# opendilab/DI-engine

Hardware: NVIDIA H100
Metric: learner transitions/sec (GAE+ppo_error fwd+bwd, T=128 x B=4096 per GPU) (higher is better)
Workload: dtype f32

## Files before the change

### di-engine_b200/_lib.py

```python
import ctypes
import os
from ctypes import c_double, c_int, c_longlong, c_size_t, c_void_p

_HERE = os.path.dirname(os.path.abspath(__file__))
LIB_PATH = os.environ.get("B200RL_LIB") or os.path.join(_HERE, "lib", "libb200rl.so")

P = c_void_p
LL = c_longlong
D = c_double
I = c_int

PROTOTYPES = {
    "b200rl_version": [],
    "b200rl_built_for_sm": [],
    "b200rl_workspace_bytes": [],
    "b200rl_gae": [P, P, P, P, P, P, LL, LL, LL, D, D, I, P],
    "b200rl_gae_returns": [P, P, P, P, P, LL, LL, LL, D, D, I, D, P, P, P, P, P, P, P, c_size_t, P],
    "b200rl_adv_stats": [P, LL, P, P, c_size_t, P],
    "b200rl_normalize": [P, P, LL, P, P],
    "b200rl_gae_returns_norm": [P, P, P, P, P, LL, LL, D, D, I, D, P, P, P, P, P, P, P, P, P, c_size_t, P],
    "b200rl_value_map_fwd": [I, P, LL, P, P],
    "b200rl_value_map_bwd": [I, P, P, LL, P, P],
    "b200rl_impala_mask": [P, P, P, LL, LL, P, P, P, P],
    "b200rl_ppo_fwd": [P, P, P, P, P, P, P, P, P, LL, LL, LL, D, I, D, I, P, P, P, P, c_size_t, P],
    "b200rl_ppo_bwd": [P, P, P, P, P, P, P, P, P, LL, LL, LL, D, I, D, I, P, P, P, P, P, P, P, P, P, P, P],
    "b200rl_ppo_fwd_grad": [P, P, P, P, P, P, P, P, P, LL, LL, LL, D, I, D, I, P, P, P, P, P, P, P, P, c_size_t, P],
    "b200rl_ppo_value_fwd": [P, P, P, P, LL, D, I, P, P, P, c_size_t, P],
    "b200rl_ppo_fused_supported": [P, P, P, P, P, P, P, P, P, P, LL, LL],
    "b200rl_ppo_tile_geometry": [LL, LL, I, I, I, I, P],
    "b200rl_qntd_fwd": [P, P, P, P, P, P, P, P, LL, P, LL, LL, LL, I, D, I, I, D, I, D, I, LL, D, P, P, P, P, P, P, P,
                        c_size_t, P],
    "b200rl_qntd_bwd": [P, P, P, P, P, LL, LL, LL, I, LL, I, P, P],
    "b200rl_dqfd_fwd": [P, P, P, P, P, P, P, P, P, P, P, LL, P, LL, LL, I, D, I, I, D, I, D, D, D, D, D, LL, D, P, P, P,
                        P, P, P, P, P, P, c_size_t, P],
    "b200rl_dqfd_bwd": [P, P, P, P, P, P, P, P, LL, LL, D, D, D, LL, I, P, P],
    "b200rl_soft_td_fwd": [I, P, P, P, P, P, P, P, P, LL, LL, LL, LL, I, D, D, D, I, I, D, P, P, P, P, P, P, P, P, P,
                           c_size_t, P],
    "b200rl_dntd_fwd":[P, P, P, P, P, P, P, LL, P, LL, P, LL, LL, LL, I, I, D, D, D, P, P, P, P, P, P, c_size_t, P],
    "b200rl_dntd_bwd": [P, P, P, P, LL, P, P, LL, LL, I, I, P, P],
    "b200rl_lambda_returns": [P, P, P, D, P, D, P, I, LL, LL, P, P],
    "b200rl_lambda_returns_bwd": [P, P, P, P, P, D, P, D, P, I, LL, LL, P, P, P, P, P],
    "b200rl_tb_cross_entropy_fwd": [P, P, P, LL, LL, LL, P, P],
    "b200rl_tb_cross_entropy_bwd": [P, P, P, P, LL, LL, LL, P, P],
    "b200rl_td_lambda_fwd": [P, P, P, D, D, LL, LL, P, P, P, c_size_t, P],
    "b200rl_scale": [P, P, P, LL, P],
    "b200rl_upgo_head_fwd": [P, P, P, P, P, P, LL, LL, LL, P, P, P, P, c_size_t, P],
    "b200rl_upgo_head_bwd": [P, P, P, P, P, LL, LL, LL, I, P, P],
    "b200rl_vtrace_fwd": [P, P, P, P, P, P, LL, LL, LL, D, D, D, D, D, P, P, P, P, P, c_size_t, P],
    "b200rl_vtrace_continuous_fwd": [P, P, P, P, P, P, P, P, LL, LL, LL, D, D, D, D, D, P, P, P, P, P, c_size_t, P],
    "b200rl_vtrace_continuous_bwd": [P, P, P, P, P, P, P, P, P, LL, LL, LL, P, P, P, P],
# ... 76 lines not shown
```

### di-engine_b200/csrc/gae_tile.cuh

```cuda
#pragma once
#include "common.cuh"

namespace b200rl {

template <int ID, int COUNT>
__device__ __forceinline__ void named_bar_sync() {
    asm volatile("bar.sync %0, %1;" ::"n"(ID), "n"(COUNT) : "memory");
}
template <int ID, int COUNT>
__device__ __forceinline__ void named_bar_arrive() {
    asm volatile("bar.arrive %0, %1;" ::"n"(ID), "n"(COUNT) : "memory");
}
template <int COUNT>
__device__ __forceinline__ void chunk_arrive(int k) {
    if (k == 0) named_bar_arrive<1, COUNT>();
    else if (k == 1) named_bar_arrive<2, COUNT>();
    else if (k == 2) named_bar_arrive<3, COUNT>();
    else named_bar_arrive<4, COUNT>();
}
__device__ __forceinline__ void scanned_arrive(int k) {
    if (k == 0) named_bar_arrive<5, 64>();
    else if (k == 1) named_bar_arrive<6, 64>();
    else if (k == 2) named_bar_arrive<7, 64>();
    else named_bar_arrive<8, 64>();
}
__device__ __forceinline__ void scanned_wait(int k) {
    if (k == 0) named_bar_sync<5, 64>();
    else if (k == 1) named_bar_sync<6, 64>();
    else if (k == 2) named_bar_sync<7, 64>();
    else named_bar_sync<8, 64>();
}
template <int COUNT>
__device__ __forceinline__ void chunk_wait(int k) {
    if (k == 0) named_bar_sync<1, COUNT>();
    else if (k == 1) named_bar_sync<2, COUNT>();
    else if (k == 2) named_bar_sync<3, COUNT>();
    else named_bar_sync<4, COUNT>();
}

constexpr int GAE_CH = 32;
constexpr int GAE_NCHUNK = 4;
constexpr int GAE_SLAB = GAE_CH * GAE_NCHUNK;

template <int TC, bool VEC, class OnChunk>
__device__ __forceinline__ void gae_tile_body(
    const float* __restrict__ value, float* __restrict__ next_value, const float* __restrict__ reward,
    const float* __restrict__ done, const float* __restrict__ traj, float* __restrict__ adv, long long T,
    long long C, long long A, float gamma, float gl, int mask_inplace, long long c0,
    float (*s_d)[GAE_CH][TC], float (*s_f)[GAE_CH][TC], OnChunk on_chunk_done, float vscale = 0.f) {
    constexpr int NL = (TC / 4) * 32;
    constexpr int NTHREADS = NL + 32;
    const long long Caux = C / A;
    const bool is_scan = threadIdx.x < 32;
    const int ltid = threadIdx.x - 32;
    float carry = 0.f;
    for (long long hi = T; hi > 0; hi -= GAE_SLAB) {
        const long long lo = hi > GAE_SLAB ? hi - GAE_SLAB : 0;
        const int rows = (int)(hi - lo);
        if (!is_scan) {
            if (VEC) {
                constexpr int TPR = TC / 4;
                const int cq = (ltid % TPR) * 4;
                const int rr = ltid / TPR;
                const long long c = c0 + cq;
                const bool col_ok = c < C;
                constexpr int DEPTH = 2;
                float4 v[DEPTH], nv[DEPTH], rw[DEPTH], dn[DEPTH], tf[DEPTH];
                auto issue = [&](int k, int b) {
                    const int r = rows - 1 - k * GAE_CH - rr;
                    if (r >= 0 && col_ok) {
                        const long long off = (lo + r) * C + c;
                        v[b] = ldg_stream4(reinterpret_cast<const float4*>(value + off));
                        nv[b] = ldg_stream4(reinterpret_cast<const float4*>(next_value + off));
                        rw[b] = ldg_stream4(reinterpret_cast<const float4*>(reward + off));
                        dn[b] = done ? ldg_stream4(reinterpret_cast<const float4*>(done + off))
                                     : make_float4(0.f, 0.f, 0.f, 0.f);
                        tf[b] = traj ? ldg_stream4(reinterpret_cast<const float4*>(traj + off)) : dn[b];
                    }
                };
#pragma unroll
                for (int k = 0; k < DEPTH; ++k) issue(k, k);
#pragma unroll
                for (int k = 0; k < GAE_NCHUNK; ++k) {
                    const int b = k % DEPTH;
                    const int r = rows - 1 - k * GAE_CH - rr;
                    if (r >= 0 && col_ok) {
                        float vv[4] = {v[b].x, v[b].y, v[b].z, v[b].w}, nn[4] = {nv[b].x, nv[b].y, nv[b].z, nv[b].w};
                        float rw4[4] = {rw[b].x, rw[b].y, rw[b].z, rw[b].w};
                        float dd[4] = {dn[b].x, dn[b].y, dn[b].z, dn[b].w};
                        float tt[4] = {tf[b].x, tf[b].y, tf[b].z, tf[b].w};
                        float de[4], fa[4];
                        bool changed = false;
#pragma unroll
                        for (int q = 0; q < 4; ++q) {
                            if (vscale != 0.f) {
                                vv[q] = fmul(vv[q], vscale);
                                nn[q] = fmul(nn[q], vscale);
                            }
                            if (done) {
                                changed |= (dd[q] != 0.f);
                                nn[q] = fmul(nn[q], fsub(1.f, dd[q]));
                            }
                            de[q] = fsub(fadd(rw4[q], fmul(gamma, nn[q])), vv[q]);
                            fa[q] = fmul(gl, fsub(1.f, tt[q]));
                        }
                        *reinterpret_cast<float4*>(&s_d[k][rr][cq]) = make_float4(de[0], de[1], de[2], de[3]);
                        *reinterpret_cast<float4*>(&s_f[k][rr][cq]) = make_float4(fa[0], fa[1], fa[2], fa[3]);
                        if (changed && mask_inplace)
                            *reinterpret_cast<float4*>(next_value + (lo + r) * C + c) =
                                make_float4(nn[0], nn[1], nn[2], nn[3]);
                    }
                    chunk_arrive<NTHREADS>(k);
                    if (k + DEPTH < GAE_NCHUNK) issue(k + DEPTH, b);
                }
            } else {
#pragma unroll
                for (int k = 0; k < GAE_NCHUNK; ++k) {
                    const int rtop = rows - 1 - k * GAE_CH;
                    for (int i = ltid; i < GAE_CH * TC; i += NL) {
                        const int rr = i / TC, cc = i % TC;
                        const int r = rtop - rr;
                        const long long c = c0 + cc;
                        if (r >= 0 && c < C) {
                            const long long off = (lo + r) * C + c;
                            const long long aoff = (lo + r) * Caux + c / A;
                            float nvv = next_value[off];
                            if (vscale != 0.f) nvv = fmul(nvv, vscale);
                            const float dnn = done ? done[aoff] : 0.f;
                            const float tff = traj ? traj[aoff] : dnn;
                            if (done) {
                                const float mm = fmul(nvv, fsub(1.f, dnn));
                                if (mask_inplace && dnn != 0.f) next_value[off] = mm;
                                nvv = mm;
                            }
                            const float vvv = vscale != 0.f ? fmul(value[off], vscale) : value[off];
                            s_d[k][rr][cc] = fsub(fadd(reward[aoff], fmul(gamma, nvv)), vvv);
                            s_f[k][rr][cc] = fmul(gl, fsub(1.f, tff));
                        }
                    }
                    chunk_arrive<NTHREADS>(k);
                }
            }
        } else {
            const int cc = threadIdx.x;
            const bool lane_ok = cc < TC && c0 + cc < C;
#pragma unroll 1
            for (int k = 0; k < GAE_NCHUNK; ++k) {
                chunk_wait<NTHREADS>(k);
                const int rtop = rows - 1 - k * GAE_CH;
                if (lane_ok && rtop >= 0) {
                    if (rtop >= GAE_CH - 1) {
                        float d[GAE_CH], f[GAE_CH];
#pragma unroll
                        for (int j = 0; j < GAE_CH; ++j) {
                            d[j] = s_d[k][j][cc];
                            f[j] = s_f[k][j][cc];
                        }
#pragma unroll
                        for (int j = 0; j < GAE_CH; ++j) {
                            carry = fadd(d[j], fmul(f[j], carry));
                            s_d[k][j][cc] = carry;
                        }
                    } else {
                        for (int j = 0; j <= rtop; ++j) {
                            carry = fadd(s_d[k][j][cc], fmul(s_f[k][j][cc], carry));
                            s_d[k][j][cc] = carry;
                        }
                    }
                }
                scanned_arrive(k);
// ... 36 lines not shown
```

### di-engine_b200/csrc/policy.cu

```cuda
#include <math.h>

#include "../../include/b200rl.h"
#include "policy_stats.cuh"

namespace b200rl {

constexpr int GS_NT = 1024;
constexpr int GS_MAX_T = 24576;

template <int VN>
__global__ void __launch_bounds__(GS_NT) gae_seq_kernel(const float* __restrict__ value, float* __restrict__ next_value,
                                                       const float* __restrict__ reward, const float* __restrict__ done,
                                                       const float* __restrict__ traj, float* __restrict__ adv, int T,
                                                       float gamma, float gl, int mask_inplace, RetArgs ra) {
    pdl_prologue();
    extern __shared__ float s_seq[];
    float* s_d = s_seq;
    float* s_f = s_seq + T;
    __shared__ int s_nseg;
    __shared__ int s_cnt[GS_NT / 32];
    const int tid = threadIdx.x;
    const float vs = ra.vscale;
    float mu = 0.f, sigma = 1.f;
    if constexpr (VN == VN_POPART) {
        mu = *ra.mu;
        sigma = *ra.sigma;
    }
    for (int t = tid; t < T; t += GS_NT) {
        const float v = vn_decode<VN>(value[t], vs);
        float nv = vn_decode<VN>(next_value[t], vs);
        float r = reward[t];
        if constexpr (VN == VN_POPART) r = __fdiv_rn(fsub(r, mu), sigma);
        const float d = done ? done[t] : 0.f;
        const float tf = traj ? traj[t] : d;
        if (done) {
// ... 132 lines not shown
            ret_one<VN>(vs, v.w, a.w, ru.w, vo.w, ro.w, acc, pv);
            if (ra.ret_unnorm) reinterpret_cast<float4*>(ra.ret_unnorm)[i] = ru;
            if (ra.value_out) reinterpret_cast<float4*>(ra.value_out)[i] = vo;
            if (ra.ret_out) reinterpret_cast<float4*>(ra.ret_out)[i] = ro;
            if (i + stride < n4) {
                v = v4[i + stride];
                a = a4[i + stride];
            }
        }
    } else {
        float v = 0.f, a = 0.f;
        if (i < n) {
            v = value[i];
            a = adv[i];
        }
        ret_pivots<VN>(vs, ret_value<VN>(ld_after_wait(value), vs), ld_after_wait(adv), pv);
        for (; i < n; i += stride) {
            float ru, vo, ro;
            ret_one<VN>(vs, v, a, ru, vo, ro, acc, pv);
            if (ra.ret_unnorm) ra.ret_unnorm[i] = ru;
            if (ra.value_out) ra.value_out[i] = vo;
            if (ra.ret_out) ra.ret_out[i] = ro;
            if (i + stride < n) {
                v = value[i + stride];
                a = adv[i + stride];
            }
        }
    }
    if (!ra.stats && !ra.adv_stats) return;
    double tot[4];
    if (stats_grid_join<4, 256>(acc, tot, ws_part, ws_join)) write_ret_stats<VN>(ra, tot, pv, (double)n);
}

__global__ void __launch_bounds__(256) adv_stats_kernel(const float* __restrict__ x, long long n, float* __restrict__ out,
                                                        double* __restrict__ ws_part, unsigned int* __restrict__ ws_join) {
    pdl_prologue();
    const double p = stats_pivot(ld_after_wait(x));
    double acc[2] = {0.0, 0.0};
    for (long long i = (long long)blockIdx.x * 256 + threadIdx.x; i < n; i += (long long)gridDim.x * 256)
        moments_add(acc[0], acc[1], x[i], p);
    double tot[2];
    if (stats_grid_join<2, 256>(acc, tot, ws_part, ws_join)) write_adv_stats(out, tot[0], tot[1], p, (double)n);
}

__global__ void __launch_bounds__(256) normalize_kernel(const float* __restrict__ x, const float* __restrict__ stats,
                                                        long long n, float* __restrict__ out) {
    pdl_prologue();
    const float m = ld_after_wait(stats), d = ld_after_wait(stats + 1);
    for (long long i = (long long)blockIdx.x * 256 + threadIdx.x; i < n; i += (long long)gridDim.x * 256)
        out[i] = __fdiv_rn(fsub(x[i], m), d);
}

__global__ void __launch_bounds__(256) impala_mask_kernel(const float* __restrict__ values, const float* __restrict__ rewards,
                                                          const float* __restrict__ done, long long T, long long B,
                                                          float* __restrict__ values_out, float* __restrict__ rewards_out,
                                                          float* __restrict__ weights_out) {
    pdl_prologue();
    const long long n = (T + 1) * B;
    for (long long i = (long long)blockIdx.x * 256 + threadIdx.x; i < n; i += (long long)gridDim.x * 256) {
        const long long t = i / B;
        const float m = t >= 1 ? fsub(1.f, done[i - B]) : 1.f;
        values_out[i] = t >= 1 ? fmul(values[i], m) : values[i];
        if (t < T) {
            if (weights_out) weights_out[i] = m;
            if (rewards_out) rewards_out[i] = fmul(rewards[i], m);
        }
// ... 21 lines not shown
        sg = *sigma;
    }
    for (long long i = (long long)blockIdx.x * 256 + threadIdx.x; i < n; i += (long long)gridDim.x * 256) {
        y0[i] = value_map<M>(x0[i], m, sg);
        if (x1) y1[i] = value_map<M>(x1[i], m, sg);
    }
}

template <int M>
__global__ void __launch_bounds__(256) value_map_bwd_kernel(const float* __restrict__ x, const float* __restrict__ g,
                                                            float* __restrict__ dx, long long n) {
    pdl_prologue();
    for (long long i = (long long)blockIdx.x * 256 + threadIdx.x; i < n; i += (long long)gridDim.x * 256) {
        const float xi = x[i], s = vn_sign(xi), gs = fmul(g[i], s);
        const float d = M == VM_SYMLOG ? __fdiv_rn(gs, fadd(fabsf(xi), 1.f)) : fmul(gs, expf(fabsf(xi)));
        dx[i] = fadd(0.f, fmul(d, s));
    }
}

}

using namespace b200rl;

namespace b200rl {
int gae_scan(const float* value, float* next_value, const float* reward, const float* done, const float* traj_flag, float* adv,
             long long T, long long C, long long A, double gamma_d, double lambda_d, int mask_next_value_inplace,
             float vscale, void* stream);
}

static double* ws_stats_part(float* ws) { return reinterpret_cast<double*>(ws + WS_CTRL_WORDS); }
static unsigned int* ws_joins(float* ws) { return reinterpret_cast<unsigned int*>(ws + WS_FX_OFF_WORDS + 48); }
static_assert(WS_CTRL_WORDS % 2 == 0 && WS_CTRL_WORDS + NUM_SMS * 8 * 4 * 2 <= WS_PARTIAL_LIMIT_WORDS,
              "the statistics rows fit the workspace's partial region");

extern "C" int b200rl_adv_stats(const float* x, long long n, float* stats2, float* workspace, size_t workspace_bytes,
                                void* stream) {
    if (!x || !stats2 || !workspace || n < 1 || workspace_bytes < WS_MIN_BYTES) return B200RL_ERR_ARG;
    long long grid = div_up(n, 256 * 8);
    if (grid > NUM_SMS * 4) grid = NUM_SMS * 4;
    if (grid < 1) grid = 1;
    return launch_k(adv_stats_kernel, (int)grid, 256, 0, (cudaStream_t)stream, x, n, stats2, ws_stats_part(workspace),
                    ws_joins(workspace));
}

extern "C" int b200rl_normalize(const float* x, const float* stats2, long long n, float* out, void* stream) {
    if (!x || !stats2 || !out || n < 0) return B200RL_ERR_ARG;
    if (n == 0) return B200RL_OK;
    long long grid = div_up(n, 256 * 4);
    if (grid > NUM_SMS * 8) grid = NUM_SMS * 8;
    return launch_k(normalize_kernel, (int)grid, 256, 0, (cudaStream_t)stream, x, stats2, n, out);
}

extern "C" int b200rl_gae_returns(const float* value, float* next_value, const float* reward, const float* done,
                                  const float* traj_flag, long long T, long long C, long long A, double gamma,
                                  double lambda_, int mask_next_value_inplace, double value_scale, float* adv,
                                  float* unnormalized_return, float* value_out, float* return_out, float* stats3,
                                  float* adv_stats2, float* workspace, size_t workspace_bytes, void* stream) {
    if (T < 1 || C < 1 || A < 1 || !value || !next_value || !reward || !adv || !workspace ||
        workspace_bytes < WS_MIN_BYTES || value_scale < 0.0)
        return B200RL_ERR_ARG;
    RetArgs ra{};
    ra.vscale = (float)value_scale;
    ra.ret_unnorm = unnormalized_return; ra.value_out = value_out; ra.ret_out = return_out; ra.stats = stats3;
    ra.adv_stats = adv_stats2;
    cudaStream_t st = (cudaStream_t)stream;
    if (C == 1 && T <= GS_MAX_T) {
        const size_t smem = (size_t)2 * T * sizeof(float);
        if (int rc = smem_opt_in<gae_seq_kernel<VN_PPO>>(smem)) return rc;
        return launch_k(gae_seq_kernel<VN_PPO>, 1, GS_NT, smem, st, value, next_value, reward, done, traj_flag, adv, (int)T,
                        (float)gamma, (float)(gamma * lambda_), mask_next_value_inplace, ra);
    }
    const bool want_epi = unnormalized_return || value_out || return_out || stats3 || adv_stats2;
    int rc = gae_scan(value, next_value, reward, done, traj_flag, adv, T, C, A, gamma, lambda_, mask_next_value_inplace,
                      (float)value_scale, stream);
    if (rc != 0 || !want_epi) return rc;
    const long long n = T * C;
    const bool vec = (n % 4 == 0) && aligned16(value) && aligned16(adv) && (!unnormalized_return || aligned16(unnormalized_return)) &&
                     (!value_out || aligned16(value_out)) && (!return_out || aligned16(return_out));
    long long grid = div_up(n, 256 * (vec ? 8 : 4));
    if (grid > NUM_SMS * 8) grid = NUM_SMS * 8;
    if (vec)
        return launch_k(returns_kernel<VN_PPO, true>, (int)grid, 256, 0, st, value, (const float*)adv, n, ra,
                        ws_stats_part(workspace), ws_joins(workspace));
    return launch_k(returns_kernel<VN_PPO, false>, (int)grid, 256, 0, st, value, (const float*)adv, n, ra,
                    ws_stats_part(workspace), ws_joins(workspace));
}

static long long map_grid(long long n) {
    long long grid = div_up(n, 256 * 4);
    if (grid > NUM_SMS * 8) grid = NUM_SMS * 8;
    return grid < 1 ? 1 : grid;
}

template <int VN>
static int launch_gae_seq(const float* value, const float* next_value, const float* reward, const float* done,
                          const float* traj_flag, float* adv, long long T, double gamma, double lambda_, const RetArgs& ra,
                          cudaStream_t st) {
    const size_t smem = (size_t)2 * T * sizeof(float);
    if (int rc = smem_opt_in<gae_seq_kernel<VN>>(smem)) return rc;
    return launch_k(gae_seq_kernel<VN>, 1, GS_NT, smem, st, value, const_cast<float*>(next_value), reward, done, traj_flag,
                    adv, (int)T, (float)gamma, (float)(gamma * lambda_), 0, ra);
}

template <int VN>
static int launch_returns(const float* value, const float* adv, long long n, const RetArgs& ra, float* workspace,
                          cudaStream_t st) {
    const bool vec = (n % 4 == 0) && aligned16(value) && aligned16(adv) && (!ra.value_out || aligned16(ra.value_out)) &&
                     (!ra.ret_out || aligned16(ra.ret_out));
// ... 111 lines not shown
```

### di-engine_b200/csrc/policy_stats.cuh

```cuda
#pragma once
#include <math.h>

#include "common.cuh"

namespace b200rl {

template <class T>
__device__ __forceinline__ T warp_sum_t(T v) {
#pragma unroll
    for (int o = 16; o > 0; o >>= 1) v += __shfl_xor_sync(0xffffffffu, v, o);
    return v;
}

template <int K, int NT>
__device__ __forceinline__ void block_sum_d(double (&v)[K], double (&tot)[K]) {
    __shared__ double s_bs[K][NT / 32];
    const int lane = threadIdx.x & 31, wid = threadIdx.x >> 5;
#pragma unroll
    for (int k = 0; k < K; ++k) {
        const double r = warp_sum_t(v[k]);
        if (lane == 0) s_bs[k][wid] = r;
    }
    __syncthreads();
    if (threadIdx.x == 0) {
// ... 44 lines not shown
__device__ __forceinline__ float vn_encode(float v, float vs) {
    if constexpr (VN == VN_PPO || VN == VN_BASELINE) return vs != 0.f ? __fdiv_rn(v, vs) : v;
    else if constexpr (VN == VN_RESCALE) return vn_h(v);
    else if constexpr (VN == VN_SYMLOG) return vn_symlog(v);
    else return v;
}

template <int VN>
__device__ __forceinline__ float ret_encode(float vs, float v, float a, float& ru, float& vo, float& ro) {
    const float r = fadd(v, a);
    ru = r;
    vo = vn_encode<VN>(v, vs);
    ro = vn_encode<VN>(r, vs);
    return VN == VN_PPO ? r : ro;
}

__device__ __forceinline__ double stats_pivot(float x0) { return isfinite(x0) ? (double)x0 : 0.0; }

__device__ __forceinline__ float ld_after_wait(const float* p) { return __ldcg(p); }

__device__ __forceinline__ void moments_add(double& s1, double& s2, float x, double p) {
    const double d = (double)x - p;
    s1 += d;
    s2 = fma(d, d, s2);
}

template <int VN>
__device__ __forceinline__ float ret_value(float v, float vs) {
    if constexpr (VN == VN_PPO || VN == VN_BASELINE) return vn_decode<VN>(v, vs);
    else return v;
}

template <int VN>
__device__ __forceinline__ void ret_one(float vs, float v, float a, float& ru, float& vo, float& ro, double (&acc)[4],
                                        const double (&pv)[2]) {
    moments_add(acc[0], acc[1], ret_encode<VN>(vs, ret_value<VN>(v, vs), a, ru, vo, ro), pv[0]);
    moments_add(acc[2], acc[3], a, pv[1]);
}

template <int VN>
__device__ __forceinline__ void ret_pivots(float vs, float v0, float a0, double (&pv)[2]) {
    float ru, vo, ro;
    pv[0] = stats_pivot(ret_encode<VN>(vs, v0, a0, ru, vo, ro));
    pv[1] = stats_pivot(a0);
}

template <int K, int NT>
__device__ __forceinline__ bool stats_grid_join(double (&acc)[K], double (&tot)[K], double* part, unsigned int* ticket) {
    __shared__ bool s_last;
    block_sum_d<K, NT>(acc, tot);
    if (gridDim.x == 1) return threadIdx.x == 0;
    if (threadIdx.x == 0) {
#pragma unroll
        for (int k = 0; k < K; ++k) part[(size_t)blockIdx.x * K + k] = tot[k];
        __threadfence();
        s_last = atomicAdd(ticket, 1u) == gridDim.x - 1;
    }
    __syncthreads();
    if (!s_last) return false;
    __threadfence();
    double v[K];
#pragma unroll
    for (int k = 0; k < K; ++k) v[k] = 0.0;
    for (unsigned int b = threadIdx.x; b < gridDim.x; b += NT)
#pragma unroll
        for (int k = 0; k < K; ++k) v[k] += __ldcg(part + (size_t)b * K + k);
    block_sum_d<K, NT>(v, tot);
    if (threadIdx.x == 0) *ticket = 0u;
    return threadIdx.x == 0;
}

__device__ __forceinline__ void write_adv_stats(float* out, double s1, double s2, double p, double nn) {
    const double d = s1 / nn;
    const double var = (s2 - s1 * d) / (nn - 1.0);
    const double sd = var != var ? var : sqrt(fmax(var, 0.0));
    out[0] = (float)(p + d);
    out[1] = fadd((float)sd, 1e-8f);
}

template <int VN>
__device__ __forceinline__ double pop_var(double v) {
    return (VN != VN_PPO && v != v) ? v : fmax(v, 0.0);
}

template <int VN>
__device__ __forceinline__ void write_ret_stats(const RetArgs& ra, const double (&tot)[4], const double (&pv)[2],
                                                double nn) {
    if (ra.stats) {
        const double d = tot[0] / nn;
        ra.stats[0] = (float)(pv[0] + d);
        ra.stats[1] = (float)pop_var<VN>(tot[1] / nn - d * d);
        ra.stats[2] = (float)nn;
    }
    if (ra.adv_stats) write_adv_stats(ra.adv_stats, tot[2], tot[3], pv[1], nn);
}

}
```

### di-engine_b200/csrc/ppo.cu

```cuda
#include "../../include/b200rl.h"
#include "ppo_math.cuh"

namespace b200rl {

constexpr int PS_CW = 8;
constexpr int PS_R = PS_CW * 32;
constexpr int PS_THREADS = PS_R + 32;
constexpr int PS_MAX_STAGES = 8;
constexpr int PS_AHEAD = 2;
constexpr size_t PS_SMEM_LIMIT = 227 * 1024 - 1024;
constexpr int PS_TRACE_STAGES = 56;

template <int NC, int WHAT>
__global__ void __launch_bounds__(PS_THREADS, 1) ppo_tile_kernel(PpoArgs a, float* ws, int n_stages, int trace) {
    extern __shared__ __align__(128) unsigned char smem[];
    unsigned long long* tr = trace ? reinterpret_cast<unsigned long long*>(ws + 65536) + blockIdx.x * 64 : nullptr;
    if (tr && threadIdx.x == 0) tr[0] = gtimer();
    pdl_prologue();
    if (tr && threadIdx.x == 0) tr[1] = gtimer();
    constexpr bool GRADS = (WHAT != PPO_FWD);
    constexpr bool LOSSES = (WHAT != PPO_BWD);
    const int N = NC ? NC : a.N;
    const int tid = threadIdx.x;
    const int wid = tid >> 5, lane = tid & 31;
    const bool has_pre = a.logit_pre != nullptr, has_w = a.weight != nullptr;
    const PpoTileLayout L = ppo_layout(N, has_pre, has_w, PS_R);
    const int NS = n_stages;
    uint64_t* full = reinterpret_cast<uint64_t*>(smem + NS * L.stage_bytes);
    uint64_t* empty = full + PS_MAX_STAGES;

    float g[4] = {0.f, 0.f, 0.f, 0.f};
    if (GRADS && upstream<4>(a.rec, WHAT == PPO_BWD, ppo_owned(a), g)) return;
    const PpoUpstream up{g[0], g[1], g[2], g[3], 1.f / (float)a.S};

    const long long n_full = a.S / PS_R;
    const int tail_rows = (int)(a.S - n_full * PS_R);
    const long long n_tiles = n_full + (tail_rows ? 1 : 0);
    const long long t0 = n_tiles * blockIdx.x / gridDim.x, t1 = n_tiles * (blockIdx.x + 1) / gridDim.x;
    const int my_n = (int)(t1 - t0);

    if (tid == 0) {
        for (int s = 0; s < NS; ++s) {
            mbar_init(&full[s], 1);
            mbar_init(&empty[s], PS_CW);
        }
        mbar_fence_init();
    }
    __syncthreads();

    float acc[6] = {0.f, 0.f, 0.f, 0.f, 0.f, 0.f};
    if (wid == PS_CW) {
        if (lane == 0) {
            for (int i = 0; i < my_n; ++i) {
                const long long t = t0 + i;
                if (t >= n_full) break;
                const int sg = i % NS;
                if (i >= NS) mbar_wait(&empty[sg], (uint32_t)(((i / NS) - 1) & 1));
                if (NS > PS_AHEAD && i >= PS_AHEAD) {
                    const int jb = i - PS_AHEAD;
                    mbar_wait(&full[jb % NS], (uint32_t)((jb / NS) & 1));
                }
                const long long row0 = t * PS_R;
                unsigned char* st = smem + sg * L.stage_bytes;
                uint64_t* bar = &full[sg];
                mbar_expect_tx(bar, (uint32_t)L.tx_bytes);
                tma_load_1d(st, a.logit_new + row0 * N, L.logit_bytes, bar);
                tma_load_1d(st + L.off_old, a.logit_old + row0 * N, L.logit_bytes, bar);
                if (has_pre) tma_load_1d(st + L.off_pre, a.logit_pre + row0 * N, L.logit_bytes, bar);
                tma_load_1d(st + L.off_act, a.action + row0, PS_R * 8, bar);
                tma_load_1d(st + L.off_vn, a.value_new + row0, PS_R * 4, bar);
                tma_load_1d(st + L.off_vo, a.value_old + row0, PS_R * 4, bar);
                tma_load_1d(st + L.off_adv, a.adv + row0, PS_R * 4, bar);
                tma_load_1d(st + L.off_ret, a.ret + row0, PS_R * 4, bar);
                if (has_w) tma_load_1d(st + L.off_w, a.weight + row0, PS_R * 4, bar);
            }
        }
    } else {
        const int rit = wid * 32 + lane;
        const int warp_out_bytes = 32 * N * 4;
        for (int i = 0; i < my_n; ++i) {
            const long long t = t0 + i;
            const long long row0 = t * PS_R;
            const int sg = i % NS;
            unsigned char* st = smem + sg * L.stage_bytes;
            const bool full_tile = t < n_full;
            if (full_tile) {
                mbar_wait(&full[sg], (uint32_t)((i / NS) & 1));
                if (tr && tid == 0) {
                    const unsigned long long now = gtimer();
                    if (i == 0) tr[2] = now;
                    tr[3] = now;
                    if (i < PS_TRACE_STAGES) tr[8 + i] = now;
                }
            } else if (rit < tail_rows) {
                float* d0 = reinterpret_cast<float*>(st) + rit * N;
                float* d1 = reinterpret_cast<float*>(st + L.off_old) + rit * N;
                float* d2 = reinterpret_cast<float*>(st + L.off_pre) + rit * N;
                for (int k = 0; k < N; ++k) {
                    d0[k] = a.logit_new[(row0 + rit) * N + k];
                    d1[k] = a.logit_old[(row0 + rit) * N + k];
                    if (has_pre) d2[k] = a.logit_pre[(row0 + rit) * N + k];
                }
                reinterpret_cast<long long*>(st + L.off_act)[rit] = a.action[row0 + rit];
                reinterpret_cast<float*>(st + L.off_vn)[rit] = a.value_new[row0 + rit];
                reinterpret_cast<float*>(st + L.off_vo)[rit] = a.value_old[row0 + rit];
                reinterpret_cast<float*>(st + L.off_adv)[rit] = a.adv[row0 + rit];
                reinterpret_cast<float*>(st + L.off_ret)[rit] = a.ret[row0 + rit];
// ... 195 lines not shown
    if (grid_sum<1, NT>(acc, tot, ws, 0) && threadIdx.x == 0) out[0] = (float)(0.5 * tot[0] / (double)S);
}

struct PsGeo {
    int grid, stages;
    size_t smem;
};
static PsGeo ps_pick(long long S, int N, bool has_pre, bool has_w, bool verify_only, int sm_count) {
    PsGeo g{};
    const size_t stage = (size_t)ppo_layout(N, has_pre, has_w, PS_R).stage_bytes;
    const size_t bars = 2 * PS_MAX_STAGES * sizeof(uint64_t);
    const long long n_tiles = (S + PS_R - 1) / PS_R;
    g.grid = (int)(n_tiles < sm_count ? n_tiles : sm_count);
    const long long per_cta = g.grid > 0 ? (n_tiles + g.grid - 1) / g.grid : 0;
    long long stages = verify_only ? 1 : (long long)((PS_SMEM_LIMIT - bars) / stage);
    if (stages > PS_MAX_STAGES) stages = PS_MAX_STAGES;
    if (stages > per_cta) stages = per_cta;
    g.stages = stages < 1 ? 0 : (int)stages;
    g.smem = (size_t)g.stages * stage + bars;
    return g;
}

template <int NC, int WHAT>
static int launch_tile(const PpoArgs& a, float* out, float* ws, size_t ws_bytes, cudaStream_t st) {
    int sm_count = 0;
    if (int rc = sm_count_of(sm_count)) return rc;
    const PsGeo g = ps_pick(a.S, a.N, a.logit_pre != nullptr, a.weight != nullptr, WHAT == PPO_BWD && a.rec.used, sm_count);
    if (g.stages < 1) return B200RL_ERR_ARG;
    constexpr auto kern = ppo_tile_kernel<NC, WHAT>;
    if (int rc = smem_opt_in<kern>(g.smem)) return rc;
    if (WHAT != PPO_BWD && !ws_partials_fit((long long)g.grid * 6, ws_bytes)) return B200RL_ERR_WORKSPACE;
    const int trace = WHAT != PPO_BWD && trace_enabled();
    if (trace && (size_t)65536 * 4 + (size_t)g.grid * 64 * 8 > ws_bytes) return B200RL_ERR_WORKSPACE;
    if (int rc = launch_k(kern, g.grid, PS_THREADS, g.smem, st, a, ws, g.stages, trace)) return rc;
    if (WHAT == PPO_BWD) return B200RL_OK;
    return launch_finalize(ws, out, ppo_finalize_args(a.S, a.logit_pre != nullptr, g.grid), st);
}

template <int WHAT>
static int dispatch_tile(const PpoArgs& a, float* out, float* ws, size_t ws_bytes, cudaStream_t st) {
    return with_nc(a.N, [&](auto nc) { return launch_tile<nc, WHAT>(a, out, ws, ws_bytes, st); });
}

}

using namespace b200rl;

static int fill_args(PpoArgs& a, const float* logit_new, const float* logit_old, const float* logit_pretrained,
                     const long long* action, const float* value_new, const float* value_old, const float* adv,
                     const float* return_, const float* weight, long long S, long long G, long long N,
                     double clip_ratio, int use_value_clip, double dual_clip, int kl_type, const float* adv_stats,
                     const float* factor) {
    a.adv_stats = adv_stats;
    a.factor = factor;
    a.logit_new = logit_new; a.logit_old = logit_old; a.logit_pre = logit_pretrained; a.action = action;
    a.value_new = value_new; a.value_old = value_old; a.adv = adv; a.ret = return_; a.weight = weight;
    a.S = S; a.G = (int)G; a.N = (int)N; a.clip = (float)clip_ratio; a.clip_lo = (float)(1.0 - clip_ratio);
    a.clip_hi = (float)(1.0 + clip_ratio); a.dual_clip = (float)dual_clip;
    a.use_value_clip = use_value_clip; a.kl_type = kl_type;
    if (S < 0 || G < 1 || N < 1) return B200RL_ERR_ARG;
    if (!logit_new || !logit_old || !action || !value_new || !value_old || !adv || !return_) return B200RL_ERR_ARG;
    if (kl_type < 1 || kl_type > 3) return B200RL_ERR_ARG;
    return B200RL_OK;
}

extern "C" int b200rl_ppo_fwd(const float* logit_new, const float* logit_old, const float* logit_pretrained,
                              const long long* action, const float* value_new, const float* value_old,
// ... 106 lines not shown
```

### include/b200rl.h

```cpp
#ifndef B200RL_H_
#define B200RL_H_

#include <stddef.h>

#ifdef __cplusplus
extern "C" {
#endif

#if defined(__GNUC__)
#define B200RL_API __attribute__((visibility("default")))
#else
#define B200RL_API
#endif

#define B200RL_ERR_ARG (-1)
#define B200RL_ERR_WORKSPACE (-2)

B200RL_API int b200rl_version(void);
B200RL_API int b200rl_built_for_sm(void);
B200RL_API size_t b200rl_workspace_bytes(void);

B200RL_API int b200rl_gae(const float* value, float* next_value, const float* reward, const float* done, const float* traj_flag,
               float* adv, long long T, long long C, long long A, double gamma, double lambda_,
               int mask_next_value_inplace, void* stream);

B200RL_API int b200rl_gae_returns(const float* value, float* next_value, const float* reward, const float* done,
                       const float* traj_flag, long long T, long long C, long long A, double gamma, double lambda_,
                       int mask_next_value_inplace, double value_scale, float* adv, float* unnormalized_return,
                       float* value_out, float* return_out, float* stats3, float* adv_stats2, float* workspace,
                       size_t workspace_bytes, void* stream);
B200RL_API int b200rl_adv_stats(const float* x, long long n, float* stats2, float* workspace, size_t workspace_bytes,
                     void* stream);
B200RL_API int b200rl_normalize(const float* x, const float* stats2, long long n, float* out, void* stream);

B200RL_API int b200rl_gae_returns_norm(const float* value, const float* next_value, const float* reward, const float* done,
                            const float* traj_flag, long long T, long long C, double gamma, double lambda_,
                            int value_norm, double std, const float* popart_mu, const float* popart_sigma, float* adv,
                            float* value_out, float* return_out, float* stats3, float* adv_stats2, float* scratch,
                            float* workspace, size_t workspace_bytes, void* stream);

B200RL_API int b200rl_value_map_fwd(int mode, const float* x, long long n, float* y, void* stream);
B200RL_API int b200rl_value_map_bwd(int mode, const float* x, const float* g, long long n, float* dx, void* stream);

B200RL_API int b200rl_impala_mask(const float* values, const float* rewards, const float* done, long long T, long long B,
                       float* values_out, float* rewards_out, float* weights_out, void* stream);

B200RL_API int b200rl_ppo_fwd(const float* logit_new, const float* logit_old, const float* logit_pretrained,
                   const long long* action, const float* value_new, const float* value_old, const float* adv,
                   const float* return_, const float* weight, long long S, long long G, long long N,
                   double clip_ratio, int use_value_clip, double dual_clip, int kl_type, const float* adv_stats,
                   const float* factor, float* out, float* workspace, size_t workspace_bytes, void* stream);
B200RL_API int b200rl_ppo_bwd(const float* logit_new, const float* logit_old, const float* logit_pretrained,
                   const long long* action, const float* value_new, const float* value_old, const float* adv,
                   const float* return_, const float* weight, long long S, long long G, long long N,
                   double clip_ratio, int use_value_clip, double dual_clip, int kl_type, const float* adv_stats,
                   const float* factor, const float* g_policy, const float* g_value, const float* g_entropy, const float* g_kl,
                   const float* g_used, float* g_hint, float* grad_logit_new, float* grad_value_new, void* stream);
B200RL_API int b200rl_ppo_fwd_grad(const float* logit_new, const float* logit_old, const float* logit_pretrained,
                        const long long* action, const float* value_new, const float* value_old, const float* adv,
                        const float* return_, const float* weight, long long S, long long G, long long N,
                        double clip_ratio, int use_value_clip, double dual_clip, int kl_type, const float* adv_stats,
                        const float* factor, const float* g_expected, float* g_used, float* out, float* grad_logit_new,
                        float* grad_value_new, float* workspace, size_t workspace_bytes, void* stream);
// ... 249 lines not shown
```

Before: 22.17 billion.

## Fuse GAE scan with returns epilogue and prefetch PPO tiles before PDL wait

Adds a tiled GAE-returns kernel that keeps value and delta slabs in shared memory and computes unnormalized returns, value/return outputs and recentred grid statistics in the same pass. This replaces a separate scan followed by a second elementwise pass over T x C. The PPO tile kernel can now issue TMA loads for inputs that do not depend on the prior kernel before griddepcontrol.wait, overlapping them with the GAE kernel's tail. The cost is more shared memory, a deeper load pipeline, and reliance on chain analysis to decide when early loads are safe.

```diff
diff --git a/di-engine_b200/_lib.py b/di-engine_b200/_lib.py
--- a/di-engine_b200/_lib.py
+++ b/di-engine_b200/_lib.py
@@ -16,6 +16,7 @@
     "b200rl_workspace_bytes": [],
     "b200rl_gae": [P, P, P, P, P, P, LL, LL, LL, D, D, I, P],
     "b200rl_gae_returns": [P, P, P, P, P, LL, LL, LL, D, D, I, D, P, P, P, P, P, P, P, c_size_t, P],
+    "b200rl_gae_returns_geometry": [LL, LL, LL, I, I, P],
     "b200rl_adv_stats": [P, LL, P, P, c_size_t, P],
     "b200rl_normalize": [P, P, LL, P, P],
     "b200rl_gae_returns_norm": [P, P, P, P, P, LL, LL, D, D, I, D, P, P, P, P, P, P, P, P, P, c_size_t, P],
diff --git a/di-engine_b200/csrc/gae_tile.cuh b/di-engine_b200/csrc/gae_tile.cuh
--- a/di-engine_b200/csrc/gae_tile.cuh
+++ b/di-engine_b200/csrc/gae_tile.cuh
@@ -42,12 +42,13 @@
 constexpr int GAE_NCHUNK = 4;
 constexpr int GAE_SLAB = GAE_CH * GAE_NCHUNK;
 
-template <int TC, bool VEC, class OnChunk>
+template <int TC, bool VEC, class OnChunk, int DEPTH = 2>
 __device__ __forceinline__ void gae_tile_body(
     const float* __restrict__ value, float* __restrict__ next_value, const float* __restrict__ reward,
     const float* __restrict__ done, const float* __restrict__ traj, float* __restrict__ adv, long long T,
     long long C, long long A, float gamma, float gl, int mask_inplace, long long c0,
-    float (*s_d)[GAE_CH][TC], float (*s_f)[GAE_CH][TC], OnChunk on_chunk_done, float vscale = 0.f) {
+    float (*s_d)[GAE_CH][TC], float (*s_f)[GAE_CH][TC], OnChunk on_chunk_done, float vscale = 0.f,
+    float (*s_v)[GAE_CH][TC] = nullptr) {
     constexpr int NL = (TC / 4) * 32;
     constexpr int NTHREADS = NL + 32;
     const long long Caux = C / A;
@@ -64,7 +65,6 @@
                 const int rr = ltid / TPR;
                 const long long c = c0 + cq;
                 const bool col_ok = c < C;
-                constexpr int DEPTH = 2;
                 float4 v[DEPTH], nv[DEPTH], rw[DEPTH], dn[DEPTH], tf[DEPTH];
                 auto issue = [&](int k, int b) {
                     const int r = rows - 1 - k * GAE_CH - rr;
@@ -106,6 +106,7 @@
                         }
                         *reinterpret_cast<float4*>(&s_d[k][rr][cq]) = make_float4(de[0], de[1], de[2], de[3]);
                         *reinterpret_cast<float4*>(&s_f[k][rr][cq]) = make_float4(fa[0], fa[1], fa[2], fa[3]);
+                        if (s_v) *reinterpret_cast<float4*>(&s_v[k][rr][cq]) = make_float4(vv[0], vv[1], vv[2], vv[3]);
                         if (changed && mask_inplace)
                             *reinterpret_cast<float4*>(next_value + (lo + r) * C + c) =
                                 make_float4(nn[0], nn[1], nn[2], nn[3]);
@@ -136,6 +137,7 @@
                             const float vvv = vscale != 0.f ? fmul(value[off], vscale) : value[off];
                             s_d[k][rr][cc] = fsub(fadd(reward[aoff], fmul(gamma, nvv)), vvv);
                             s_f[k][rr][cc] = fmul(gl, fsub(1.f, tff));
+                            if (s_v) s_v[k][rr][cc] = vvv;
                         }
                     }
                     chunk_arrive<NTHREADS>(k);
diff --git a/di-engine_b200/csrc/policy.cu b/di-engine_b200/csrc/policy.cu
--- a/di-engine_b200/csrc/policy.cu
+++ b/di-engine_b200/csrc/policy.cu
@@ -1,6 +1,7 @@
 #include <math.h>
 
 #include "../../include/b200rl.h"
+#include "gae_tile.cuh"
 #include "policy_stats.cuh"
 
 namespace b200rl {
@@ -199,6 +200,90 @@
     if (stats_grid_join<4, 256>(acc, tot, ws_part, ws_join)) write_ret_stats<VN>(ra, tot, pv, (double)n);
 }
 
+constexpr int GR_DEPTH = 4;
+constexpr int GR_TRACE_WORD = 131072;
+
+template <int TC>
+__global__ void __launch_bounds__((TC / 4 + 1) * 32) gae_returns_tile_kernel(
+    const float* __restrict__ value, float* __restrict__ next_value, const float* __restrict__ reward,
+    const float* __restrict__ done, const float* __restrict__ traj, float* __restrict__ adv, long long T, long long C,
+    float gamma, float gl, int mask_inplace, RetArgs ra, double* __restrict__ ws_part, unsigned int* __restrict__ ws_join,
+    unsigned long long* __restrict__ trace) {
+    constexpr int NT = (TC / 4 + 1) * 32;
+    unsigned long long* tr = trace ? trace + (size_t)blockIdx.x * 8 : nullptr;
+    if (tr && threadIdx.x == 0) tr[0] = gtimer();
+    asm volatile("griddepcontrol.wait;" ::: "memory");
+    asm volatile("griddepcontrol.launch_dependents;" ::: "memory");
+    if (tr && threadIdx.x == 0) tr[1] = gtimer();
+    extern __shared__ __align__(16) float s_gr[];
+    auto s_d = reinterpret_cast<float (*)[GAE_CH][TC]>(s_gr);
+    auto s_f = s_d + GAE_NCHUNK;
+    auto s_v = s_f + GAE_NCHUNK;
+    __shared__ double s_q[2];
+    const float vs = ra.vscale;
+    const long long c0 = (long long)blockIdx.x * TC;
+    const int lane = threadIdx.x & 31;
+    const int rows_last = (int)(T - (T - 1) / GAE_SLAB * GAE_SLAB);
+    const int k_last = (rows_last - 1) / GAE_CH, r_last = (rows_last - 1) % GAE_CH;
+    double acc[4] = {0.0, 0.0, 0.0, 0.0}, q[2] = {0.0, 0.0};
+    auto epilogue = [&](long long g, bool any) {
+            const int k = (int)(g % GAE_NCHUNK);
+            const long long hi = T - g / GAE_NCHUNK * GAE_SLAB;
+            const long long lo = hi > GAE_SLAB ? hi - GAE_SLAB : 0;
+            if (g < GAE_NCHUNK) {
+                ret_pivots<VN_PPO>(vs, s_v[0][0][0], s_d[0][0][0], q);
+                if (g == 0 && lane == 0) {
+                    s_q[0] = q[0];
+                    s_q[1] = q[1];
+                }
+            }
+            if (!any) return;
+            const int rtop = (int)(hi - lo) - 1 - k * GAE_CH;
+            constexpr int TPR = TC / 4;
+            for (int i = lane; i < GAE_CH * TPR; i += 32) {
+                const int rr = i / TPR, cq = (i % TPR) * 4;
+                const int r = rtop - rr;
+                if (r >= 0 && c0 + cq < C) {
+                    const float4 a4 = *reinterpret_cast<const float4*>(&s_d[k][rr][cq]);
+                    const float4 v4 = *reinterpret_cast<const float4*>(&s_v[k][rr][cq]);
+                    float4 ru, vo, ro;
+                    ret_one_decoded<VN_PPO>(vs, v4.x, a4.x, ru.x, vo.x, ro.x, acc, q);
+                    ret_one_decoded<VN_PPO>(vs, v4.y, a4.y, ru.y, vo.y, ro.y, acc, q);
+                    ret_one_decoded<VN_PPO>(vs, v4.z, a4.z, ru.z, vo.z, ro.z, acc, q);
+                    ret_one_decoded<VN_PPO>(vs, v4.w, a4.w, ru.w, vo.w, ro.w, acc, q);
+                    const long long off = (lo + r) * C + c0 + cq;
+                    if (ra.ret_unnorm) stg_stream4(reinterpret_cast<float4*>(ra.ret_unnorm + off), ru);
+                    if (ra.value_out) stg_stream4(reinterpret_cast<float4*>(ra.value_out + off), vo);
+                    if (ra.ret_out) stg_stream4(reinterpret_cast<float4*>(ra.ret_out + off), ro);
+                }
+            }
+            if (tr && lane == 0) {
+                if (g == 0) tr[2] = gtimer();
+                if (lo == 0 && k == k_last) tr[3] = gtimer();
+            }
+        };
+    gae_tile_body<TC, true, decltype(epilogue), GR_DEPTH>(value, next_value, reward, done, traj, adv, T, C, 1, gamma, gl,
+                                                          mask_inplace, c0, s_d, s_f, epilogue, vs, s_v);
+    if (ra.stats || ra.adv_stats) {
+        double p[2] = {0.0, 0.0}, tot[4], pv[2];
+        const double n_cta = (double)T * (double)(C - c0 < TC ? C - c0 : TC);
+        __syncthreads();
+        if (threadIdx.x == 0) {
+            q[0] = s_q[0];
+            q[1] = s_q[1];
+            if (blockIdx.x == 0) ret_pivots<VN_PPO>(vs, s_v[k_last][r_last][0], s_d[k_last][r_last][0], p);
+        }
+        if (stats_grid_join_recentred<NT>(acc, q, n_cta, p, ws_part, ws_join, tot, pv)) {
+            write_ret_stats<VN_PPO>(ra, tot, pv, (double)T * (double)C);
+            if (tr) tr[6] = gtimer();
+        }
+    }
+    if (tr && threadIdx.x == 0) {
+        tr[4] = gtimer();
+        tr[5] = (unsigned long long)smid() << 32 | (unsigned long long)((T + GAE_CH - 1) / GAE_CH);
+    }
+}
+
 __global__ void __launch_bounds__(256) adv_stats_kernel(const float* __restrict__ x, long long n, float* __restrict__ out,
                                                         double* __restrict__ ws_part, unsigned int* __restrict__ ws_join) {
     pdl_prologue();
@@ -286,6 +371,42 @@
 static unsigned int* ws_joins(float* ws) { return reinterpret_cast<unsigned int*>(ws + WS_FX_OFF_WORDS + 48); }
 static_assert(WS_CTRL_WORDS % 2 == 0 && WS_CTRL_WORDS + NUM_SMS * 8 * 4 * 2 <= WS_PARTIAL_LIMIT_WORDS,
               "the statistics rows fit the workspace's partial region");
+
+template <auto K>
+static int gr_opt_in(size_t smem) {
+    static size_t opted[MAX_DEVICES];
+    int dev = 0;
+    if (int rc = current_device(dev)) return rc;
+    if (smem <= opted[dev]) return B200RL_OK;
+    if (int rc = cuda_rc(cudaFuncSetAttribute(K, cudaFuncAttributeMaxDynamicSharedMemorySize, (int)smem))) return rc;
+    opted[dev] = smem;
+    return B200RL_OK;
+}
+
+struct GrGeo {
+    int tc, grid, threads;
+    size_t smem;
+};
+static GrGeo gr_pick(long long T, long long C, long long A, bool aligned, int sm_count) {
+    GrGeo g{};
+    if (T < 1 || A != 1 || C < 4 || C % 4 != 0 || !aligned || sm_count < 1) return g;
+    const int tc = (C + 15) / 16 >= sm_count - sm_count / 16 ? 16 : 8;
+    const long long grid = (C + tc - 1) / tc;
+    if (!ws_partials_fit(grid * 8 * 2 + 4, WS_MIN_BYTES)) return g;
+    g.tc = tc;
+    g.grid = (int)grid;
+    g.threads = (tc / 4 + 1) * 32;
+    g.smem = (size_t)3 * GAE_NCHUNK * GAE_CH * tc * sizeof(float);
+    return g;
+}
+
+extern "C" int b200rl_gae_returns_geometry(long long T, long long C, long long A, int aligned, int sm_count,
+                                           long long* geometry4) {
+    if (!geometry4) return B200RL_ERR_ARG;
+    const GrGeo g = gr_pick(T, C, A, aligned != 0, sm_count);
+    geometry4[0] = g.tc; geometry4[1] = g.grid; geometry4[2] = g.threads; geometry4[3] = (long long)g.smem;
+    return B200RL_OK;
+}
 
 extern "C" int b200rl_adv_stats(const float* x, long long n, float* stats2, float* workspace, size_t workspace_bytes,
                                 void* stream) {
@@ -325,9 +446,52 @@
                         (float)gamma, (float)(gamma * lambda_), mask_next_value_inplace, ra);
     }
     const bool want_epi = unnormalized_return || value_out || return_out || stats3 || adv_stats2;
+    if (!want_epi)
+        return gae_scan(value, next_value, reward, done, traj_flag, adv, T, C, A, gamma, lambda_, mask_next_value_inplace,
+                        (float)value_scale, stream);
+    int sm_count = 0;
+    if (int rc = sm_count_of(sm_count)) return rc;
+    const bool al = aligned16(value) && aligned16(next_value) && aligned16(reward) && aligned16(adv) &&
+                    (!done || aligned16(done)) && (!traj_flag || aligned16(traj_flag)) &&
+                    (!unnormalized_return || aligned16(unnormalized_return)) && (!value_out || aligned16(value_out)) &&
+                    (!return_out || aligned16(return_out));
+    const GrGeo g = gr_pick(T, C, A, al, sm_count);
+    if (g.tc) {
+        const ChainPoint at = capture_now(st);
+        const bool trace = trace_enabled();
+        if (trace && ((long long)WS_CTRL_WORDS + (long long)g.grid * 16 + 4 > GR_TRACE_WORD ||
+                      (size_t)GR_TRACE_WORD * 4 + (size_t)g.grid * 8 * 8 > workspace_bytes))
+            return B200RL_ERR_WORKSPACE;
+        unsigned long long* tr = trace ? reinterpret_cast<unsigned long long*>(workspace + GR_TRACE_WORD) : nullptr;
+        const float gm = (float)gamma, gl = (float)(gamma * lambda_);
+        int rc;
+        if (g.tc == 16) {
+            if ((rc = gr_opt_in<gae_returns_tile_kernel<16>>(g.smem))) return rc;
+            rc = launch_k(gae_returns_tile_kernel<16>, g.grid, g.threads, g.smem, st, value, next_value, reward, done,
+                          traj_flag, adv, T, C, gm, gl, mask_next_value_inplace, ra, ws_stats_part(workspace),
+                          ws_joins(workspace), tr);
+        } else {
+            if ((rc = gr_opt_in<gae_returns_tile_kernel<8>>(g.smem))) return rc;
+            rc = launch_k(gae_returns_tile_kernel<8>, g.grid, g.threads, g.smem, st, value, next_value, reward, done,
+                          traj_flag, adv, T, C, gm, gl, mask_next_value_inplace, ra, ws_stats_part(workspace),
+                          ws_joins(workspace), tr);
+        }
+        if (rc) return rc;
+        const long long F = T * C * 4;
+        const ByteSpan w[] = {byte_span(adv, F),
+                              byte_span(unnormalized_return, F),
+                              byte_span(value_out, F),
+                              byte_span(return_out, F),
+                              byte_span(mask_next_value_inplace ? next_value : nullptr, F),
+                              byte_span(stats3, 3 * sizeof(float)),
+                              byte_span(adv_stats2, 2 * sizeof(float)),
+                              byte_span(workspace, (long long)workspace_bytes)};
+        chain_report(st, at, true, w, (int)(sizeof(w) / sizeof(w[0])));
+        return B200RL_OK;
+    }
     int rc = gae_scan(value, next_value, reward, done, traj_flag, adv, T, C, A, gamma, lambda_, mask_next_value_inplace,
                       (float)value_scale, stream);
-    if (rc != 0 || !want_epi) return rc;
+    if (rc != 0) return rc;
     const long long n = T * C;
     const bool vec = (n % 4 == 0) && aligned16(value) && aligned16(adv) && (!unnormalized_return || aligned16(unnormalized_return)) &&
                      (!value_out || aligned16(value_out)) && (!return_out || aligned16(return_out));
diff --git a/di-engine_b200/csrc/policy_stats.cuh b/di-engine_b200/csrc/policy_stats.cuh
--- a/di-engine_b200/csrc/policy_stats.cuh
+++ b/di-engine_b200/csrc/policy_stats.cuh
@@ -100,10 +100,16 @@
 }
 
 template <int VN>
+__device__ __forceinline__ void ret_one_decoded(float vs, float v, float a, float& ru, float& vo, float& ro,
+                                                double (&acc)[4], const double (&pv)[2]) {
+    moments_add(acc[0], acc[1], ret_encode<VN>(vs, v, a, ru, vo, ro), pv[0]);
+    moments_add(acc[2], acc[3], a, pv[1]);
+}
+
+template <int VN>
 __device__ __forceinline__ void ret_one(float vs, float v, float a, float& ru, float& vo, float& ro, double (&acc)[4],
                                         const double (&pv)[2]) {
-    moments_add(acc[0], acc[1], ret_encode<VN>(vs, ret_value<VN>(v, vs), a, ru, vo, ro), pv[0]);
-    moments_add(acc[2], acc[3], a, pv[1]);
+    ret_one_decoded<VN>(vs, ret_value<VN>(v, vs), a, ru, vo, ro, acc, pv);
 }
 
 template <int VN>
@@ -134,6 +140,47 @@
 #pragma unroll
         for (int k = 0; k < K; ++k) v[k] += __ldcg(part + (size_t)b * K + k);
     block_sum_d<K, NT>(v, tot);
+    if (threadIdx.x == 0) *ticket = 0u;
+    return threadIdx.x == 0;
+}
+
+template <int NT>
+__device__ __forceinline__ bool stats_grid_join_recentred(double (&acc)[4], const double (&q)[2], double n,
+                                                          const double (&p)[2], double* part, unsigned int* ticket,
+                                                          double (&tot)[4], double (&pv)[2]) {
+    __shared__ bool s_last;
+    block_sum_d<4, NT>(acc, tot);
+    if (threadIdx.x == 0) {
+        double* row = part + (size_t)blockIdx.x * 8;
+#pragma unroll
+        for (int k = 0; k < 4; ++k) row[k] = tot[k];
+        row[4] = q[0];
+        row[5] = q[1];
+        row[6] = n;
+        if (blockIdx.x == 0) {
+            part[(size_t)gridDim.x * 8] = p[0];
+            part[(size_t)gridDim.x * 8 + 1] = p[1];
+        }
+        __threadfence();
+        s_last = atomicAdd(ticket, 1u) == gridDim.x - 1;
+    }
+    __syncthreads();
+    if (!s_last) return false;
+    __threadfence();
+    pv[0] = __ldcg(part + (size_t)gridDim.x * 8);
+    pv[1] = __ldcg(part + (size_t)gridDim.x * 8 + 1);
+    double v[4] = {0.0, 0.0, 0.0, 0.0};
+    for (unsigned int b = threadIdx.x; b < gridDim.x; b += NT) {
+        const double* row = part + (size_t)b * 8;
+        const double s1r = __ldcg(row), s2r = __ldcg(row + 1), s1a = __ldcg(row + 2), s2a = __ldcg(row + 3);
+        const double nb = __ldcg(row + 6);
+        const double dr = __ldcg(row + 4) - pv[0], da = __ldcg(row + 5) - pv[1];
+        v[0] += fma(nb, dr, s1r);
+        v[1] += fma(nb * dr, dr, fma(2.0 * dr, s1r, s2r));
+        v[2] += fma(nb, da, s1a);
+        v[3] += fma(nb * da, da, fma(2.0 * da, s1a, s2a));
+    }
+    block_sum_d<4, NT>(v, tot);
     if (threadIdx.x == 0) *ticket = 0u;
     return threadIdx.x == 0;
 }
diff --git a/di-engine_b200/csrc/ppo.cu b/di-engine_b200/csrc/ppo.cu
--- a/di-engine_b200/csrc/ppo.cu
+++ b/di-engine_b200/csrc/ppo.cu
@@ -8,16 +8,24 @@
 constexpr int PS_THREADS = PS_R + 32;
 constexpr int PS_MAX_STAGES = 8;
 constexpr int PS_AHEAD = 2;
+constexpr int PS_EARLY = 4;
 constexpr size_t PS_SMEM_LIMIT = 227 * 1024 - 1024;
 constexpr int PS_TRACE_STAGES = 56;
 
 template <int NC, int WHAT>
-__global__ void __launch_bounds__(PS_THREADS, 1) ppo_tile_kernel(PpoArgs a, float* ws, int n_stages, int trace) {
+__global__ void __launch_bounds__(PS_THREADS, 1) ppo_tile_kernel(PpoArgs a, float* ws, int n_stages, int trace,
+                                                                 int early) {
     extern __shared__ __align__(128) unsigned char smem[];
     unsigned long long* tr = trace ? reinterpret_cast<unsigned long long*>(ws + 65536) + blockIdx.x * 64 : nullptr;
     if (tr && threadIdx.x == 0) tr[0] = gtimer();
-    pdl_prologue();
-    if (tr && threadIdx.x == 0) tr[1] = gtimer();
+    const bool early_path = WHAT != PPO_BWD && early > 0;
+    if (!early_path) {
+        pdl_prologue();
+        if (tr && threadIdx.x == 0) {
+            tr[1] = gtimer();
+            tr[6] = 0;
+        }
+    }
     constexpr bool GRADS = (WHAT != PPO_FWD);
     constexpr bool LOSSES = (WHAT != PPO_BWD);
     const int N = NC ? NC : a.N;
@@ -30,8 +38,7 @@
     uint64_t* empty = full + PS_MAX_STAGES;
 
     float g[4] = {0.f, 0.f, 0.f, 0.f};
-    if (GRADS && upstream<4>(a.rec, WHAT == PPO_BWD, ppo_owned(a), g)) return;
-    const PpoUpstream up{g[0], g[1], g[2], g[3], 1.f / (float)a.S};
+    if (!early_path && GRADS && upstream<4>(a.rec, WHAT == PPO_BWD, ppo_owned(a), g)) return;
 
     const long long n_full = a.S / PS_R;
     const int tail_rows = (int)(a.S - n_full * PS_R);
@@ -39,19 +46,57 @@
     const long long t0 = n_tiles * blockIdx.x / gridDim.x, t1 = n_tiles * (blockIdx.x + 1) / gridDim.x;
     const int my_n = (int)(t1 - t0);
 
-    if (tid == 0) {
-        for (int s = 0; s < NS; ++s) {
-            mbar_init(&full[s], 1);
-            mbar_init(&empty[s], PS_CW);
-        }
-        mbar_fence_init();
-    }
-    __syncthreads();
+    auto issue = [&](int i, bool first_part, bool second_part) {
+        const long long row0 = (t0 + i) * PS_R;
+        unsigned char* st = smem + (i % NS) * L.stage_bytes;
+        uint64_t* bar = &full[i % NS];
+        if (first_part) {
+            mbar_expect_tx(bar, (uint32_t)L.tx_bytes);
+            tma_load_1d(st, a.logit_new + row0 * N, L.logit_bytes, bar);
+            tma_load_1d(st + L.off_old, a.logit_old + row0 * N, L.logit_bytes, bar);
+            if (has_pre) tma_load_1d(st + L.off_pre, a.logit_pre + row0 * N, L.logit_bytes, bar);
+            tma_load_1d(st + L.off_act, a.action + row0, PS_R * 8, bar);
+            tma_load_1d(st + L.off_vn, a.value_new + row0, PS_R * 4, bar);
+        }
+        if (second_part) {
+            tma_load_1d(st + L.off_vo, a.value_old + row0, PS_R * 4, bar);
+            tma_load_1d(st + L.off_adv, a.adv + row0, PS_R * 4, bar);
+            tma_load_1d(st + L.off_ret, a.ret + row0, PS_R * 4, bar);
+        }
+        if (first_part && has_w) tma_load_1d(st + L.off_w, a.weight + row0, PS_R * 4, bar);
+    };
+    auto init_ring = [&] {
+        if (tid == 0) {
+            for (int s = 0; s < NS; ++s) {
+                mbar_init(&full[s], 1);
+                mbar_init(&empty[s], PS_CW);
+            }
+            mbar_fence_init();
+        }
+        __syncthreads();
+    };
+    const int n_early = !early_path ? 0 : min(min(early, NS), (int)(n_full - t0 < my_n ? n_full - t0 : my_n));
+    if (early_path) {
+        asm volatile("griddepcontrol.launch_dependents;" ::: "memory");
+        init_ring();
+        if (wid == PS_CW && lane == 0)
+            for (int i = 0; i < n_early; ++i) issue(i, true, false);
+        asm volatile("griddepcontrol.wait;" ::: "memory");
+        if (tr && threadIdx.x == 0) {
+            tr[1] = gtimer();
+            tr[6] = (unsigned long long)(n_early > 0 ? n_early : 0);
+        }
+        if (GRADS) upstream<4>(a.rec, false, ppo_owned(a), g);
+    } else {
+        init_ring();
+    }
+    const PpoUpstream up{g[0], g[1], g[2], g[3], 1.f / (float)a.S};
 
     float acc[6] = {0.f, 0.f, 0.f, 0.f, 0.f, 0.f};
     if (wid == PS_CW) {
         if (lane == 0) {
-            for (int i = 0; i < my_n; ++i) {
+            for (int i = 0; i < n_early; ++i) issue(i, false, true);
+            for (int i = n_early; i < my_n; ++i) {
                 const long long t = t0 + i;
                 if (t >= n_full) break;
                 const int sg = i % NS;
@@ -60,19 +105,7 @@
                     const int jb = i - PS_AHEAD;
                     mbar_wait(&full[jb % NS], (uint32_t)((jb / NS) & 1));
                 }
-                const long long row0 = t * PS_R;
-                unsigned char* st = smem + sg * L.stage_bytes;
-                uint64_t* bar = &full[sg];
-                mbar_expect_tx(bar, (uint32_t)L.tx_bytes);
-                tma_load_1d(st, a.logit_new + row0 * N, L.logit_bytes, bar);
-                tma_load_1d(st + L.off_old, a.logit_old + row0 * N, L.logit_bytes, bar);
-                if (has_pre) tma_load_1d(st + L.off_pre, a.logit_pre + row0 * N, L.logit_bytes, bar);
-                tma_load_1d(st + L.off_act, a.action + row0, PS_R * 8, bar);
-                tma_load_1d(st + L.off_vn, a.value_new + row0, PS_R * 4, bar);
-                tma_load_1d(st + L.off_vo, a.value_old + row0, PS_R * 4, bar);
-                tma_load_1d(st + L.off_adv, a.adv + row0, PS_R * 4, bar);
-                tma_load_1d(st + L.off_ret, a.ret + row0, PS_R * 4, bar);
-                if (has_w) tma_load_1d(st + L.off_w, a.weight + row0, PS_R * 4, bar);
+                issue(i, true, true);
             }
         }
     } else {
@@ -334,7 +367,15 @@
     if (WHAT != PPO_BWD && !ws_partials_fit((long long)g.grid * 6, ws_bytes)) return B200RL_ERR_WORKSPACE;
     const int trace = WHAT != PPO_BWD && trace_enabled();
     if (trace && (size_t)65536 * 4 + (size_t)g.grid * 64 * 8 > ws_bytes) return B200RL_ERR_WORKSPACE;
-    if (int rc = launch_k(kern, g.grid, PS_THREADS, g.smem, st, a, ws, g.stages, trace)) return rc;
+    int early = 0;
+    if (WHAT != PPO_BWD) {
+        const ChainPoint at = capture_now(st);
+        const long long S = a.S, L = S * a.N * 4;
+        const ByteSpan r[] = {byte_span(a.logit_new, L), byte_span(a.logit_old, L), byte_span(a.logit_pre, L),
+                              byte_span(a.action, S * 8), byte_span(a.value_new, S * 4), byte_span(a.weight, S * 4)};
+        if (chain_may_defer(st, at, r, (int)(sizeof(r) / sizeof(r[0])))) early = PS_EARLY;
+    }
+    if (int rc = launch_k(kern, g.grid, PS_THREADS, g.smem, st, a, ws, g.stages, trace, early)) return rc;
     if (WHAT == PPO_BWD) return B200RL_OK;
     return launch_finalize(ws, out, ppo_finalize_args(a.S, a.logit_pre != nullptr, g.grid), st);
 }
diff --git a/include/b200rl.h b/include/b200rl.h
--- a/include/b200rl.h
+++ b/include/b200rl.h
@@ -29,6 +29,8 @@
                        int mask_next_value_inplace, double value_scale, float* adv, float* unnormalized_return,
                        float* value_out, float* return_out, float* stats3, float* adv_stats2, float* workspace,
                        size_t workspace_bytes, void* stream);
+B200RL_API int b200rl_gae_returns_geometry(long long T, long long C, long long A, int aligned, int sm_count,
+                                           long long* geometry4);
 B200RL_API int b200rl_adv_stats(const float* x, long long n, float* stats2, float* workspace, size_t workspace_bytes,
                      void* stream);
 B200RL_API int b200rl_normalize(const float* x, const float* stats2, long long n, float* out, void* stream);
```

Result: no change. 22.12 billion, median of 6 (-0.2%).
